# rlangefe/pygemma

Hardware: AMD Instinct MI355X
Metric: SNPs/sec (whole node) at n=10,000 c=5; K-eigendecomp wallclock (higher is better)
Workload: dtype i8x3->i32 MFMA (genotype codes exact, integer accumulation exact; U as 24-bit fixed point per eigenvector in three int8 planes) rotation + f64 Gram/sweeps (f32 rounding points of the reference)

## Files before the change

### pygemma_amd/csrc/assoc.hip

```cpp
#include "common.hpp"

#include <cmath>

namespace pg {

constexpr int NLAM = 11;
#ifndef PG_ASSOC_WPB
#define PG_ASSOC_WPB 2
#endif
constexpr int WPB = PG_ASSOC_WPB;
#define PG_MINV 1e-35f
#ifndef PG_FUSE_PQ_MAX
#define PG_FUSE_PQ_MAX 36
#endif
#ifndef PG_FUSE_PQR_MAX
#define PG_FUSE_PQR_MAX 28
#endif
#ifndef PG_PFD
#define PG_PFD 2
#endif
#ifndef PG_CHUNK_MIN_NP
#define PG_CHUNK_MIN_NP 80
#endif
#ifndef PG_SCAN_NV
#define PG_SCAN_NV 96
#endif
#ifndef PG_SWEEP_LDS_MIN_SLOTS
#define PG_SWEEP_LDS_MIN_SLOTS 3
#endif
#ifndef PG_PHENO_SPLIT_XE
#define PG_PHENO_SPLIT_XE 26
#endif
#ifndef PG_WAVES
#define PG_WAVES 2
#endif
#ifndef PG_ASSOC_FINAL_P
#define PG_ASSOC_FINAL_P 1
#endif
#ifndef PG_ASSOC_NEWTON_REUSE
#define PG_ASSOC_NEWTON_REUSE 1
#endif
#ifndef PG_REUSE_MAX_SLOTS
#define PG_REUSE_MAX_SLOTS 4
#endif
#ifndef PG_ASSOC_DECADE_HOIST
#define PG_ASSOC_DECADE_HOIST 1
#endif

__host__ __device__ constexpr size_t assoc_dtab_doubles(int c) { return (size_t)c * (c + 2) * 4 + 8; }

__host__ __device__ constexpr size_t assoc_sav_doubles(int sav_slots) { return sav_slots ? (size_t)2 * (2 * sav_slots + 1) * 64 : 0; }
__host__ __device__ constexpr size_t assoc_per_wave_bytes(int M, bool sweep_lds, int sav_slots, size_t evalout_bytes, int n_vals)
{
    return (((sweep_lds ? (size_t)3 * M * 8 : 0) + assoc_sav_doubles(sav_slots) * 8 + (size_t)NLAM * 2 * M * 8 + NLAM * evalout_bytes + 2 * NLAM * 4 +
             (size_t)n_vals * 4) + 15) & ~(size_t)15;
}

struct AssocParams {
    int n, npad, c, niter, nu, grid, rowf;
    long long p, ldx;
    const float *xr;
    const float *fixed;
    float *htab;
    double *fixg;
    double *t1tab;
    float *ldHtab;
    double *dtab;
    float lam11[NLAM];
    float logl_c;
    const int *leaf, *node, *level, *chunk;
    int n_leaf, n_level, n_chunk, n_vals;
    float *beta, *se, *tau, *lam;
    double *F;
    unsigned long long *stats;
    unsigned *trace;
    unsigned long long *passes;
    int lrt, nhalf;
    float ml_c;
    float *lalt, *lamalt;
    const double *xbuf;
    int xe, xcol;
};

struct EvalOut { float yPy, yPPy, yPPPy, trP, trPP, ld, Pxx_c, Pyx_c, sh, shh; };

__device__ __forceinline__ float hinv_f32(float lam, float d)
// ... 349 lines not shown
{
    const float4 *src = reinterpret_cast<const float4 *>(pr.fixed + (size_t)i * pr.rowf);
#pragma unroll
    for (int k = 0; k < Elem<C>::S4; k++) e.row[k] = src[k];
    const int ic = min(i, pr.n - 1);
    e.x = HASX ? xrow[ic] : 0.0f;
}
constexpr int PFD = PG_PFD;
template <class E, int PF = PFD, class LoadF, class BodyF>
__device__ __forceinline__ void pipelined(int niter, LoadF &&ld, BodyF &&body)
{
    E buf[PF];
#pragma unroll
    for (int d = 0; d < PF; d++) ld(buf[d], d < niter ? d : niter - 1);
    for (int it = 0; it < niter; it += PF) {
#pragma unroll
        for (int d = 0; d < PF; d++) {
            if (it + d < niter) body(buf[d], it + d);
            const int nx = it + d + PF;
            ld(buf[d], nx < niter ? nx : niter - 1);
        }
    }
}
template <int C>
__device__ __forceinline__ void unpack_elem(const AssocParams &pr, const Elem<C> &e, int i, float &d, float (&col)[C + 2])
{
    float buf[4 * Elem<C>::S4];
#pragma unroll
    for (int k = 0; k < Elem<C>::S4; k++) {
        buf[4 * k] = e.row[k].x; buf[4 * k + 1] = e.row[k].y; buf[4 * k + 2] = e.row[k].z; buf[4 * k + 3] = e.row[k].w;
    }
    d = buf[0];
#pragma unroll
    for (int j = 0; j < C; j++) col[j] = buf[1 + j];
    col[C] = e.x;
    col[C + 1] = buf[C + 1];
}
template <int C> struct WaldElem {
    using E = Elem<C>;
    using Row = const float *;
    template <bool HASX>
    static __device__ __forceinline__ void load(const AssocParams &pr, Row xrow, int i, E &e) { load_elem<C, HASX>(pr, xrow, i, e); }
    static __device__ __forceinline__ void unpack(const AssocParams &pr, const E &e, int i, float &d, float (&col)[C + 2]) { unpack_elem<C>(pr, e, i, d, col); }
};

template <int C, int MASK, bool HASX, class EL = WaldElem<C>>
__device__ __forceinline__ void gram_pass(const AssocParams &pr, typename EL::Row xrow, float lam, int lane, float *htab_out,
                                          double (&Po)[Shape<C>::SLOTS], double (&Qo)[Shape<C>::SLOTS], double (&Ro)[Shape<C>::SLOTS],
                                          double &t1, double &t2)
{
    constexpr int M = Shape<C>::M, NP = Shape<C>::NP;
    constexpr bool DP = (MASK & 1) != 0, DQ = (MASK & 2) != 0, DR = (MASK & 4) != 0;
    double P[DP ? NP : 1], Q[DQ ? NP : 1], R[DR ? NP : 1];
#pragma unroll
    for (int k = 0; k < NP; k++) { if constexpr (DP) P[k] = 0.0; if constexpr (DQ) Q[k] = 0.0; if constexpr (DR) R[k] = 0.0; }
    double s1 = 0.0, s2 = 0.0;
    using E = typename EL::E;
    pipelined<E>(pr.niter, [&](E &e, int it) { EL::template load<HASX>(pr, xrow, it * 64 + lane, e); },
                       [&](const E &cur, int it) {
        const int i = it * 64 + lane;
        float d, colf[M];
        EL::unpack(pr, cur, i, d, colf);
        const float h = hinv_f32(lam, d);
        if (htab_out) htab_out[i] = h;
        const double hd = (double)h;
        double col[M], a[M];
#pragma unroll
        for (int j = 0; j < M; j++) { col[j] = (double)colf[j]; a[j] = hd * col[j]; }
        if (DP || DQ) {
#pragma unroll
            for (int j = 0; j < M; j++)
#pragma unroll
                for (int k = 0; k <= j; k++) {
                    if constexpr (DP) P[tri(j, k)] = fma(a[j], col[k], P[tri(j, k)]);
                    if constexpr (DQ) Q[tri(j, k)] = fma(a[j], a[k], Q[tri(j, k)]);
                }
        }
        if (DP) s1 += hd;
        if constexpr (DR) {
            const double h2 = hd * hd;
#pragma unroll
            for (int j = 0; j < M; j++) {
                const double gj = h2 * col[j];
#pragma unroll
                for (int k = 0; k <= j; k++) R[tri(j, k)] = fma(gj, a[k], R[tri(j, k)]);
            }
            s2 = fma(hd, hd, s2);
        }
    });
    if constexpr (DP) { scatter_entries<C>(P, lane, Po); t1 = bfly(s1); }
    if constexpr (DQ) scatter_entries<C>(Q, lane, Qo);
    if constexpr (DR) { scatter_entries<C>(R, lane, Ro); t2 = bfly(s2); }
}

template <int C, int PW, int SL, bool HASX, class EL = WaldElem<C>>
__device__ __forceinline__ void gram_pass_slot(const AssocParams &pr, typename EL::Row xrow, float lam, int lane, float *htab_out, double &out, double &tsum)
{
    constexpr int M = Shape<C>::M, E0 = 64 * SL, NV = Shape<C>::slot_nv(SL), NVP = next_pow2(NV);
    double acc[NVP];
#pragma unroll
    for (int k = 0; k < NVP; k++) acc[k] = 0.0;
    double s = 0.0;
    using E = typename EL::E;
    pipelined<E, (M > 22 ? 1 : PFD)>(pr.niter, [&](E &e, int it) { EL::template load<HASX>(pr, xrow, it * 64 + lane, e); },
                       [&](const E &cur, int it) {
        const int i = it * 64 + lane;
        float d, colf[M];
        EL::unpack(pr, cur, i, d, colf);
        const float h = hinv_f32(lam, d);
        if (htab_out) htab_out[i] = h;
        const double hd = (double)h, h2 = hd * hd;
        double col[M], a[M], g[PW == 3 ? M : 1];
#pragma unroll
        for (int j = 0; j < M; j++) { col[j] = (double)colf[j]; a[j] = hd * col[j]; if constexpr (PW == 3) g[j] = h2 * col[j]; }
#pragma unroll
        for (int j = 0; j < M; j++)
#pragma unroll
            for (int k = 0; k <= j; k++) {
                const int e = tri(j, k);
                if (e >= E0 && e < E0 + NV) {
                    if constexpr (PW == 1) acc[e - E0] = fma(a[j], col[k], acc[e - E0]);
                    else if constexpr (PW == 2) acc[e - E0] = fma(a[j], a[k], acc[e - E0]);
                    else acc[e - E0] = fma(g[j], a[k], acc[e - E0]);
                }
            }
        if constexpr (SL == 0 && PW == 1) s += hd;
        if constexpr (SL == 0 && PW == 3) s = fma(hd, hd, s);
    });
    out = reduce_scatter<NVP>(acc, lane);
    if constexpr (SL == 0 && (PW == 1 || PW == 3)) tsum = bfly(s);
}
template <int C, int PW, bool HASX, int SL = 0, class EL = WaldElem<C>>
__device__ __forceinline__ void slot_passes(const AssocParams &pr, typename EL::Row xrow, float lam, int lane, float *htab_out,
                                            double (&X)[Shape<C>::SLOTS], double &tsum)
{
    gram_pass_slot<C, PW, SL, HASX, EL>(pr, xrow, lam, lane, SL == 0 ? htab_out : nullptr, X[SL], tsum);
    if constexpr (SL + 1 < Shape<C>::SLOTS) slot_passes<C, PW, HASX, SL + 1, EL>(pr, xrow, lam, lane, htab_out, X, tsum);
}

template <int C, int MASK, class EL = WaldElem<C>>
__device__ __forceinline__ void gram_powers(const AssocParams &pr, typename EL::Row xrow, float lam, int lane,
                                            double (&P)[Shape<C>::SLOTS], double (&Q)[Shape<C>::SLOTS], double (&R)[Shape<C>::SLOTS],
                                            double &t1, double &t2)
{
    constexpr bool DP = (MASK & 1) != 0, DQ = (MASK & 2) != 0, DR = (MASK & 4) != 0;
    if constexpr (Shape<C>::CHUNKED) {
        double tq = 0.0;
        if constexpr (DP) slot_passes<C, 1, true, 0, EL>(pr, xrow, lam, lane, nullptr, P, t1);
        if constexpr (DQ) slot_passes<C, 2, true, 0, EL>(pr, xrow, lam, lane, nullptr, Q, tq);
        if constexpr (DR) slot_passes<C, 3, true, 0, EL>(pr, xrow, lam, lane, nullptr, R, t2);
    } else if constexpr (MASK == PW_PQR && Shape<C>::FUSE_PQR) {
        gram_pass<C, 7, true, EL>(pr, xrow, lam, lane, nullptr, P, Q, R, t1, t2);
    } else if constexpr (DP && DQ && Shape<C>::FUSE_PQ) {
        gram_pass<C, 3, true, EL>(pr, xrow, lam, lane, nullptr, P, Q, R, t1, t2);
        if constexpr (DR) gram_pass<C, 4, true, EL>(pr, xrow, lam, lane, nullptr, P, Q, R, t1, t2);
    } else {
        if constexpr (DP) gram_pass<C, 1, true, EL>(pr, xrow, lam, lane, nullptr, P, Q, R, t1, t2);
        if constexpr (DQ) gram_pass<C, 2, true, EL>(pr, xrow, lam, lane, nullptr, P, Q, R, t1, t2);
        if constexpr (DR) gram_pass<C, 4, true, EL>(pr, xrow, lam, lane, nullptr, P, Q, R, t1, t2);
// ... 4 lines not shown
__device__ __forceinline__ void eval_specific(const AssocParams &pr, typename EL::Row xrow, float lam, int lane, const Own<C> &own, EvalOut &o,
                                              double *piv)
{
    constexpr int SLOTS = Shape<C>::SLOTS;
    double P[SLOTS], Q[SLOTS], R[SLOTS], t1 = 0.0, t2 = 0.0;
#pragma unroll
    for (int sl = 0; sl < SLOTS; sl++) { Q[sl] = 0.0; R[sl] = 0.0; }
    gram_powers<C, PW, EL>(pr, xrow, lam, lane, P, Q, R, t1, t2);
    lane_sweeps<C, PW>(P, Q, R, own, t1, t2, lane, o, piv);
}

template <int C>
__global__ __launch_bounds__(64) void setup_tabs_kernel(AssocParams pr)
{
    constexpr int NP = Shape<C>::NP, SLOTS = Shape<C>::SLOTS;
    extern __shared__ float smem_f[];
    const int t = blockIdx.x, lane = threadIdx.x;
    const float lam = pr.lam11[t];
    Own<C> own;
    own.init(lane);
    double P[SLOTS], Q[SLOTS], R[SLOTS], t1 = 0.0, t2 = 0.0;
    if constexpr (Shape<C>::CHUNKED) {
        double tq = 0.0;
        slot_passes<C, 1, false>(pr, nullptr, lam, lane, pr.htab + (size_t)t * pr.npad, P, t1);
        slot_passes<C, 2, false>(pr, nullptr, lam, lane, nullptr, Q, tq);
    } else if constexpr (Shape<C>::FUSE_PQ) {
        gram_pass<C, 3, false>(pr, nullptr, lam, lane, pr.htab + (size_t)t * pr.npad, P, Q, R, t1, t2);
    } else {
        gram_pass<C, 1, false>(pr, nullptr, lam, lane, pr.htab + (size_t)t * pr.npad, P, Q, R, t1, t2);
        gram_pass<C, 2, false>(pr, nullptr, lam, lane, nullptr, P, Q, R, t1, t2);
    }
#pragma unroll
    for (int sl = 0; sl < SLOTS; sl++)
        if (own.valid[sl]) {
            pr.fixg[((size_t)t * 2 + 0) * NP + own.e[sl]] = P[sl];
            pr.fixg[((size_t)t * 2 + 1) * NP + own.e[sl]] = Q[sl];
        }
    float ldH = device_logdet_H(pr, lam, lane, smem_f);
    if (lane == 0) { pr.t1tab[t] = t1; pr.ldHtab[t] = ldH; }
    if constexpr (PG_ASSOC_DECADE_HOIST && C >= 1) {
        __shared__ double piv_s[Shape<C>::SWEEP_LDS ? 3 * Shape<C>::M : 1];
        if (pr.dtab) {
            double *rec = pr.dtab + (size_t)t * assoc_dtab_doubles(C);
            EvalOut e;
            lane_sweeps<C, PW_PQ, true>(P, Q, R, own, t1, 0.0, lane, e, piv_s, rec);
            double *tail = rec + (size_t)C * Shape<C>::M * 4;
            if (lane == 0) { tail[4] = t1; tail[5] = (double)ldH; tail[6] = (double)lam; tail[7] = 0.0; }
        }
    }
}

template <int C, int GG>
__device__ __forceinline__ void scan_accumulate(const AssocParams &pr, const float *xrow, int t0, int lane, double *xent)
{
    constexpr int M = Shape<C>::M, NV = GG * 2 * M;
    constexpr int NV0 = NV < 64 ? NV : 64, NV1 = NV > 64 ? NV - 64 : 0;
    constexpr int NVP0 = next_pow2(NV0), NVP1 = next_pow2(NV1 > 0 ? NV1 : 1);
    static_assert(NV <= 128, "scan group too large");
    double acc[NV0 == 64 ? 64 + NVP1 : NVP0];
#pragma unroll
    for (int k = 0; k < (NV0 == 64 ? 64 + NVP1 : NVP0); k++) acc[k] = 0.0;
    struct SE { Elem<C> e; float h[GG]; };
    pipelined<SE>(pr.niter, [&](SE &q, int it) {
        const int i = it * 64 + lane;
        load_elem<C>(pr, xrow, i, q.e);
#pragma unroll
        for (int g = 0; g < GG; g++) q.h[g] = pr.htab[(size_t)(t0 + g) * pr.npad + i];
    }, [&](const SE &q, int it) {
        const int i = it * 64 + lane;
        float d, colf[M];
        unpack_elem<C>(pr, q.e, i, d, colf);
        const double xd = (double)colf[C];
        double z[M];
#pragma unroll
        for (int k = 0; k <= C; k++) z[k] = xd * (double)colf[k];
        z[C + 1] = (double)colf[C + 1] * xd;
#pragma unroll
        for (int g = 0; g < GG; g++) {
            const double hd = (double)q.h[g];
            const double h2 = hd * hd;
#pragma unroll
            for (int k = 0; k <= C + 1; k++) {
                acc[g * 2 * M + k] = fma(hd, z[k], acc[g * 2 * M + k]);
                acc[g * 2 * M + M + k] = fma(h2, z[k], acc[g * 2 * M + M + k]);
            }
        }
    });
    {
        double t[NVP0];
#pragma unroll
        for (int k = 0; k < NVP0; k++) t[k] = acc[k];
        const double tot = reduce_scatter<NVP0>(t, lane);
        const int idx = lane % NVP0;
        if (idx < NV0 && lane < NVP0) xent[t0 * 2 * M + idx] = tot;
    }
    if constexpr (NV1 > 0) {
        double t[NVP1];
#pragma unroll
        for (int k = 0; k < NVP1; k++) t[k] = acc[64 + k];
        const double tot = reduce_scatter<NVP1>(t, lane);
        const int idx = lane % NVP1;
        if (idx < NV1 && lane < NVP1) xent[t0 * 2 * M + 64 + idx] = tot;
    }
}
template <int C, int T0>
__device__ __forceinline__ void scan_all(const AssocParams &pr, const float *xrow, int lane, double *xent)
{
    constexpr int G = Shape<C>::G;
    if constexpr (T0 < NLAM) {
        constexpr int GG = (NLAM - T0) < G ? (NLAM - T0) : G;
        scan_accumulate<C, GG>(pr, xrow, T0, lane, xent);
        scan_all<C, T0 + GG>(pr, xrow, lane, xent);
    }
}

template <int C, int TC, int GG, int PWS, int PW0>
__device__ __forceinline__ void scan_pheno_accumulate(const AssocParams &pr, const float *xrow, const float *Y, long long ldy, int tcn,
                                                      int t0, int lane, double *out)
{
    constexpr int M = Shape<C>::M, XE = C + 1 + TC, NV = GG * PWS * XE;
    auto dest = [&](int v) { const int gg = v / (PWS * XE), r = v - gg * PWS * XE; return (t0 + gg) * 2 * XE + PW0 * XE + r; };
    constexpr int NV0 = NV < 64 ? NV : 64, NV1 = NV > 64 ? NV - 64 : 0;
    constexpr int NVP0 = next_pow2(NV0), NVP1 = next_pow2(NV1 > 0 ? NV1 : 1);
    static_assert(NV <= 128, "scan group too large");
    double acc[NV0 == 64 ? 64 + NVP1 : NVP0];
#pragma unroll
    for (int k = 0; k < (NV0 == 64 ? 64 + NVP1 : NVP0); k++) acc[k] = 0.0;
    struct SE { Elem<C> e; float y[TC]; float h[GG]; };
    pipelined<SE>(pr.niter, [&](SE &q, int it) {
        const int i = it * 64 + lane;
        load_elem<C>(pr, xrow, i, q.e);
#pragma unroll
        for (int j = 0; j < TC; j++) q.y[j] = (i < pr.n && j < tcn) ? Y[(size_t)j * ldy + i] : 0.0f;
#pragma unroll
        for (int g = 0; g < GG; g++) q.h[g] = pr.htab[(size_t)(t0 + g) * pr.npad + i];
    }, [&](const SE &q, int it) {
        const int i = it * 64 + lane;
        float d, colf[M];
        unpack_elem<C>(pr, q.e, i, d, colf);
        const double xd = (double)colf[C];
        double z[XE];
#pragma unroll
        for (int k = 0; k <= C; k++) z[k] = xd * (double)colf[k];
#pragma unroll
        for (int j = 0; j < TC; j++) z[C + 1 + j] = (double)q.y[j] * xd;
#pragma unroll
        for (int g = 0; g < GG; g++) {
            const double hd = (double)q.h[g];
            const double h2 = hd * hd;
#pragma unroll
            for (int k = 0; k < XE; k++) {
                if constexpr (PWS == 2) {
                    acc[g * 2 * XE + k] = fma(hd, z[k], acc[g * 2 * XE + k]);
                    acc[g * 2 * XE + XE + k] = fma(h2, z[k], acc[g * 2 * XE + XE + k]);
                } else {
                    acc[g * XE + k] = fma(PW0 == 0 ? hd : h2, z[k], acc[g * XE + k]);
                }
            }
// ... 5 lines not shown
        for (int k = 0; k < NVP0; k++) t[k] = acc[k];
        const double tot = reduce_scatter<NVP0>(t, lane);
        const int idx = lane % NVP0;
        if (idx < NV0 && lane < NVP0) out[dest(idx)] = tot;
    }
    if constexpr (NV1 > 0) {
        double t[NVP1];
#pragma unroll
        for (int k = 0; k < NVP1; k++) t[k] = acc[64 + k];
        const double tot = reduce_scatter<NVP1>(t, lane);
        const int idx = lane % NVP1;
        if (idx < NV1 && lane < NVP1) out[dest(64 + idx)] = tot;
    }
}
template <int C, int TC, int T0>
__device__ __forceinline__ void scan_pheno_all(const AssocParams &pr, const float *xrow, const float *Y, long long ldy, int tcn, int lane,
                                               double *out)
{
    constexpr int XE = C + 1 + TC, PWS = XE > PG_PHENO_SPLIT_XE ? 1 : 2;
    constexpr int G0 = PWS == 1 ? 1 : (Shape<C>::SCAN_NV - XE) / (PWS * XE), G = G0 < 1 ? 1 : (G0 > NLAM ? NLAM : G0);
    if constexpr (T0 < NLAM) {
        constexpr int GG = (NLAM - T0) < G ? (NLAM - T0) : G;
        if constexpr (PWS == 2) {
            scan_pheno_accumulate<C, TC, GG, 2, 0>(pr, xrow, Y, ldy, tcn, T0, lane, out);
        } else {
            scan_pheno_accumulate<C, TC, GG, 1, 0>(pr, xrow, Y, ldy, tcn, T0, lane, out);
            scan_pheno_accumulate<C, TC, GG, 1, 1>(pr, xrow, Y, ldy, tcn, T0, lane, out);
        }
        scan_pheno_all<C, TC, T0 + GG>(pr, xrow, Y, ldy, tcn, lane, out);
    }
}
constexpr int SCAN_WPB = 4;
template <int C, int TC>
__global__ __launch_bounds__(64 * SCAN_WPB, PG_WAVES) void scan_pheno_kernel(AssocParams pr, const float *Y, long long ldy, int tcn, double *xbuf)
{
    const int wave = threadIdx.x >> 6, lane = threadIdx.x & 63;
    const long long g = (long long)blockIdx.x * SCAN_WPB + wave;
    if (g >= pr.p) return;
    scan_pheno_all<C, TC, 0>(pr, pr.xr + (size_t)g * pr.ldx, Y, ldy, tcn, lane, xbuf + (size_t)g * NLAM * 2 * (C + 1 + TC));
}

__device__ __forceinline__ void wave_lds_sync()
{
    __builtin_amdgcn_fence(__ATOMIC_RELEASE, "wavefront");
    __builtin_amdgcn_wave_barrier();
    __builtin_amdgcn_fence(__ATOMIC_ACQUIRE, "wavefront");
}

template <class Fn>
__device__ __forceinline__ double brentq_dev(Fn &&f, double xa, double xb, double fa, double fb, int maxiter = 100)
// ... 316 lines not shown
            atomicAdd(&pr.passes[2], (unsigned long long)n_full); atomicAdd(&pr.passes[3], (unsigned long long)n_reuse);
        }
    }
    ASSOC_STAMP(3);
}

#if defined(PG_ASSOC_PART) && (PG_ASSOC_PART == 6 || PG_ASSOC_PART == 7)
struct GxeRows { const float *x, *xe; };
template <int CS> struct GxeVals {
    static constexpr int S4 = (CS + 2 + 3) / 4;
    float4 row[S4];
    float x, xe;
};
template <int C> struct GxeElem {
    static constexpr int CS = C - 1;
    using E = GxeVals<CS>;
    using Row = GxeRows;
    template <bool HASX>
    static __device__ __forceinline__ void load(const AssocParams &pr, Row r, int i, E &e)
    {
        const float4 *src = reinterpret_cast<const float4 *>(pr.fixed + (size_t)i * pr.rowf);
#pragma unroll
        for (int k = 0; k < E::S4; k++) e.row[k] = src[k];
        const int ic = min(i, pr.n - 1);
        e.x = r.x[ic];
        e.xe = r.xe[ic];
    }
    static __device__ __forceinline__ void unpack(const AssocParams &pr, const E &e, int i, float &d, float (&col)[C + 2])
    {
        float buf[4 * E::S4];
#pragma unroll
        for (int k = 0; k < E::S4; k++) {
            buf[4 * k] = e.row[k].x; buf[4 * k + 1] = e.row[k].y; buf[4 * k + 2] = e.row[k].z; buf[4 * k + 3] = e.row[k].w;
        }
        d = buf[0];
#pragma unroll
        for (int j = 0; j < CS; j++) col[j] = buf[1 + j];
        col[CS] = e.x;
        col[CS + 1] = e.xe;
        col[CS + 2] = buf[CS + 1];
    }
};
template <int CS> struct GxeShape {
    static constexpr int C = CS + 1, NE = 2 * CS + 5;
    static constexpr int PWS = NE > PG_PHENO_SPLIT_XE ? 1 : 2;
    static constexpr int G0 = (Shape<C>::SCAN_NV - NE) / (PWS * NE), G = G0 < 1 ? 1 : (G0 > NLAM ? NLAM : G0);
};
__host__ __device__ constexpr size_t gxe_per_wave_bytes(int M, bool sweep_lds, int NE, size_t evalout_bytes, int n_vals)
{
    return (((sweep_lds ? (size_t)3 * M * 8 : 0) + (size_t)NLAM * 2 * NE * 8 + NLAM * evalout_bytes + 2 * NLAM * 4 + (size_t)n_vals * 4) + 15) & ~(size_t)15;
}

template <int CS, int GG, int PWS, int PW0>
__device__ __forceinline__ void gxe_scan_accumulate(const AssocParams &pr, GxeRows xr, int t0, int lane, double *out)
{
    using EL = GxeElem<CS + 1>;
    constexpr int M = CS + 3, NE = GxeShape<CS>::NE, NV = GG * PWS * NE;
    auto dest = [&](int v) { const int gg = v / (PWS * NE), r = v - gg * PWS * NE; return (t0 + gg) * 2 * NE + PW0 * NE + r; };
    constexpr int NV0 = NV < 64 ? NV : 64, NV1 = NV > 64 ? NV - 64 : 0;
    constexpr int NVP0 = next_pow2(NV0), NVP1 = next_pow2(NV1 > 0 ? NV1 : 1);
    static_assert(NV <= 128, "scan group too large");
    double acc[NV0 == 64 ? 64 + NVP1 : NVP0];
#pragma unroll
    for (int k = 0; k < (NV0 == 64 ? 64 + NVP1 : NVP0); k++) acc[k] = 0.0;
    struct SE { typename EL::E e; float h[GG]; };
    pipelined<SE>(pr.niter, [&](SE &q, int it) {
        const int i = it * 64 + lane;
        EL::template load<true>(pr, xr, i, q.e);
#pragma unroll
        for (int g = 0; g < GG; g++) q.h[g] = pr.htab[(size_t)(t0 + g) * pr.npad + i];
    }, [&](const SE &q, int it) {
        const int i = it * 64 + lane;
        float d, colf[M];
        EL::unpack(pr, q.e, i, d, colf);
        const double xd = (double)colf[CS], ed = (double)colf[CS + 1], yd = (double)colf[CS + 2];
        double z[NE];
#pragma unroll
        for (int k = 0; k < CS; k++) { z[k] = xd * (double)colf[k]; z[CS + 1 + k] = ed * (double)colf[k]; }
        z[CS] = xd * xd;
        z[2 * CS + 1] = ed * xd;
        z[2 * CS + 2] = ed * ed;
        z[2 * CS + 3] = yd * xd;
        z[2 * CS + 4] = yd * ed;
#pragma unroll
        for (int g = 0; g < GG; g++) {
            const double hd = (double)q.h[g];
            const double h2 = hd * hd;
#pragma unroll
            for (int k = 0; k < NE; k++) {
                if constexpr (PWS == 2) {
                    acc[g * 2 * NE + k] = fma(hd, z[k], acc[g * 2 * NE + k]);
                    acc[g * 2 * NE + NE + k] = fma(h2, z[k], acc[g * 2 * NE + NE + k]);
                } else {
                    acc[g * NE + k] = fma(PW0 == 0 ? hd : h2, z[k], acc[g * NE + k]);
                }
            }
        }
// ... 2 lines not shown
        double t[NVP0];
#pragma unroll
        for (int k = 0; k < NVP0; k++) t[k] = acc[k];
        const double tot = reduce_scatter<NVP0>(t, lane);
        const int idx = lane % NVP0;
        if (idx < NV0 && lane < NVP0) out[dest(idx)] = tot;
    }
    if constexpr (NV1 > 0) {
        double t[NVP1];
#pragma unroll
        for (int k = 0; k < NVP1; k++) t[k] = acc[64 + k];
        const double tot = reduce_scatter<NVP1>(t, lane);
        const int idx = lane % NVP1;
        if (idx < NV1 && lane < NVP1) out[dest(64 + idx)] = tot;
    }
}
template <int CS, int T0>
__device__ __forceinline__ void gxe_scan_all(const AssocParams &pr, GxeRows xr, int lane, double *xent)
{
    constexpr int G = GxeShape<CS>::G;
    if constexpr (T0 < NLAM) {
        constexpr int GG = (NLAM - T0) < G ? (NLAM - T0) : G;
        if constexpr (GxeShape<CS>::PWS == 2) {
            gxe_scan_accumulate<CS, GG, 2, 0>(pr, xr, T0, lane, xent);
        } else {
            gxe_scan_accumulate<CS, GG, 1, 0>(pr, xr, T0, lane, xent);
            gxe_scan_accumulate<CS, GG, 1, 1>(pr, xr, T0, lane, xent);
        }
        gxe_scan_all<CS, T0 + GG>(pr, xr, lane, xent);
    }
}

template <int CS>
__global__ __launch_bounds__(64 * WPB, PG_WAVES) void assoc_gxe_kernel(AssocParams pr, const float *xer, long long ldxe)
{
    constexpr int C = CS + 1, M = Shape<C>::M, SLOTS = Shape<C>::SLOTS, NE = GxeShape<CS>::NE, NPS = Shape<CS>::NP;
    using EL = GxeElem<C>;
    extern __shared__ unsigned char smem[];
    const int wave = threadIdx.x >> 6, lane = threadIdx.x & 63;
    const long long g = (long long)blockIdx.x * WPB + wave;
    if (g >= pr.p) return;
    constexpr size_t piv_bytes = Shape<C>::SWEEP_LDS ? (size_t)3 * M * 8 : 0;
    unsigned char *base = smem + (size_t)wave * gxe_per_wave_bytes(M, Shape<C>::SWEEP_LDS, NE, sizeof(EvalOut), pr.n_vals);
    double *piv = reinterpret_cast<double *>(base);
    base += piv_bytes;
    double *xent = reinterpret_cast<double *>(base);
    EvalOut *evs = reinterpret_cast<EvalOut *>(base + (size_t)NLAM * 2 * NE * 8);
    float *d1s = reinterpret_cast<float *>(evs + NLAM);
    float *lls = d1s + NLAM;
    float *vals = lls + NLAM;
// ... 529 lines not shown
    {
        float r = (float)((double)(n / 2) * std::log((double)n / (2.0 * M_PI)));
        pr.ml_c = r - (float)(n / 2);
    }
    pr.leaf = ctx->plan.d_leaf; pr.node = ctx->plan.d_node; pr.level = ctx->plan.d_level; pr.chunk = ctx->plan.d_chunk;
    pr.n_leaf = ctx->plan.n_leaf; pr.n_level = ctx->plan.n_level; pr.n_chunk = ctx->plan.n_chunk;
    pr.n_vals = ctx->plan.n_leaf + ctx->plan.n_node;
}

static int assoc_run(pg_ctx *ctx, int64_t n, int c, int64_t p, const float *d, const float *Wr, int64_t ldw, const float *yr,
                     const float *Xr, int64_t ldx, int grid, float *beta, float *se, float *tau, float *lambda, double *F,
                     unsigned long long *stats_dev, bool lrt, float *lalt, float *lamalt)
{
    PG_HIP(hipSetDevice(ctx->device));
    int rc = build_npsum_plan(ctx, n);
    if (rc) return rc;

    AssocParams pr{};
    fill_params(ctx, n, c, grid, pr);
    pr.p = p; pr.ldx = ldx; pr.xr = Xr;
    const int M = c + 2, NP = M * (M + 1) / 2;
    rc = ensure(ctx, &ctx->fixed, &ctx->fixed_bytes, (size_t)pr.npad * pr.rowf * 4);
    if (rc) return rc;
    const size_t off_fixg = ((size_t)NLAM * pr.npad * 4 + 255) & ~(size_t)255;
    const size_t off_t1 = off_fixg + (size_t)NLAM * 2 * NP * 8;
    const size_t off_ldh = off_t1 + NLAM * 8;
    const size_t off_dtab = (off_ldh + NLAM * 4 + 255) & ~(size_t)255;
    rc = ensure(ctx, &ctx->tabs, &ctx->tabs_bytes, off_dtab + NLAM * assoc_dtab_doubles(c) * 8 + 256);
    if (rc) return rc;
    if (!ctx->stats) PG_HIP(hipMalloc(&ctx->stats, 16));
    pr.fixed = (const float *)ctx->fixed;
    pr.htab = (float *)ctx->tabs;
    pr.fixg = (double *)((char *)ctx->tabs + off_fixg);
    pr.t1tab = (double *)((char *)ctx->tabs + off_t1);
    pr.ldHtab = (float *)((char *)ctx->tabs + off_ldh);
    pr.dtab = (double *)((char *)ctx->tabs + off_dtab);
    pr.lrt = lrt ? 1 : 0;
    pr.lalt = lalt; pr.lamalt = lamalt;
    pr.beta = beta; pr.se = se; pr.tau = tau; pr.lam = lambda; pr.F = F;
    pr.stats = stats_dev;
    pr.trace = lrt ? nullptr : ctx->eval_trace;
    pr.passes = lrt ? nullptr : ctx->pass_stats;

    build_fixed_kernel<<<(pr.npad + 255) / 256, 256, 0, ctx->stream>>>(pr.n, pr.npad, c, (int)ldw, pr.rowf, d, Wr, yr, (float *)ctx->fixed);
    PG_HIP(hipGetLastError());
    return launch_assoc_any(ctx, pr);
}

extern "C" int pg_assoc_dev(pg_ctx *ctx, int64_t n, int c, int64_t p, const float *d, const float *Wr, const float *yr,
                            const float *Xr, int64_t ldx, int grid, float *beta, float *se, float *tau, float *lambda,
                            double *F, double *pval, unsigned long long *stats_dev)
{
    PG_REQUIRE(ctx && d && Wr && yr && Xr && beta && se && tau && lambda && F, "pg_assoc_dev: NULL argument");
    PG_REQUIRE(n >= 2 && n < (1LL << 30) && p >= 0 && ldx >= n, "pg_assoc_dev: bad shape n=%lld p=%lld ldx=%lld", (long long)n, (long long)p, (long long)ldx);
    if (c < 1 || c > PG_MAX_COVARIATES) {
// ... 1 lines not shown
        return PG_ENOTSUP;
    }
    PG_REQUIRE(n - c - 1 > 0, "pg_assoc_dev: n - c - 1 must be positive");
    if (p == 0) return PG_OK;
    int rc = assoc_run(ctx, n, c, p, d, Wr, c, yr, Xr, ldx, grid, beta, se, tau, lambda, F, stats_dev, false, nullptr, nullptr);
    if (rc) return rc;
    if (pval) return pg_fdist_sf_dev(ctx, p, F, (double)(n - c - 1), pval);
    return PG_OK;
}

extern "C" int pg_assoc_warm(pg_ctx *ctx, int64_t n, int c)
{
    PG_REQUIRE(ctx && n >= 2 && n < (1LL << 30), "pg_assoc_warm: bad arguments");
    if (c < 1 || c > PG_MAX_COVARIATES) {
        set_error("pg_assoc_warm: c=%d covariates not supported by this build (1..%d)", c, PG_MAX_COVARIATES);
        return PG_ENOTSUP;
    }
    PG_HIP(hipSetDevice(ctx->device));
    int rc = build_npsum_plan(ctx, n);
    if (rc) return rc;
    const int npad = (int)((n + 63) / 64 * 64), rowf = ((c + 2 + 3) / 4) * 4, M = c + 2, NP = M * (M + 1) / 2;
    rc = ensure(ctx, &ctx->fixed, &ctx->fixed_bytes, (size_t)npad * rowf * 4);
    if (rc) return rc;
    const size_t off_fixg = ((size_t)NLAM * npad * 4 + 255) & ~(size_t)255;
    rc = ensure(ctx, &ctx->tabs, &ctx->tabs_bytes,
                ((off_fixg + (size_t)NLAM * 2 * NP * 8 + NLAM * 8 + NLAM * 4 + 255) & ~(size_t)255) + NLAM * assoc_dtab_doubles(c) * 8 + 256);
    if (rc) return rc;
    if (!ctx->stats) PG_HIP(hipMalloc(&ctx->stats, 16));
    return PG_OK;
}

extern "C" int pg_assoc_set_eval_trace(pg_ctx *ctx, unsigned *trace_dev)
{
    PG_REQUIRE(ctx, "pg_assoc_set_eval_trace: NULL ctx");
    ctx->eval_trace = trace_dev;
    return PG_OK;
}

extern "C" int pg_assoc_set_pass_stats(pg_ctx *ctx, unsigned long long *dev4)
{
    PG_REQUIRE(ctx, "pg_assoc_set_pass_stats: NULL ctx");
    ctx->pass_stats = dev4;
    return PG_OK;
}

#ifdef PG_ASSOC_STAMPS
extern "C" int pgx_assoc_stamps(long long *out4096)
{
    return hipMemcpyFromSymbol(out4096, HIP_SYMBOL(pg::g_assoc_stamps), sizeof(long long) * 4096) == hipSuccess ? 0 : -1;
}
#endif

struct PhenoLayout {
    int npad, rowf, NP, tpad_max;
    long long ptile;
    size_t off_htab, off_fixg, off_t1, off_ldh, off_xbuf, bytes;
};
static PhenoLayout pheno_layout(int64_t n, int c, int t, int64_t p)
{
    PhenoLayout L{};
    auto up = [](size_t v) { return (v + 255) & ~(size_t)255; };
    L.npad = (int)((n + 63) / 64 * 64); L.rowf = ((c + 2 + 3) / 4) * 4; L.NP = (c + 2) * (c + 3) / 2;
    const int tc = t < PHENO_CHUNK ? t : PHENO_CHUNK;
    L.tpad_max = 1;
    while (L.tpad_max < tc) L.tpad_max <<= 1;
    const size_t per_snp = (size_t)NLAM * 2 * (c + 1 + L.tpad_max) * 8;
    const long long cap = (long long)((256u << 20) / per_snp);
    L.ptile = p < cap ? p : (cap < 1024 ? 1024 : cap);
    if (L.ptile > p) L.ptile = p;
    L.off_htab = up((size_t)PHENO_CHUNK * L.npad * L.rowf * 4);
    L.off_fixg = L.off_htab + up((size_t)NLAM * L.npad * 4);
    L.off_t1 = L.off_fixg + up((size_t)PHENO_CHUNK * NLAM * 2 * L.NP * 8);
    L.off_ldh = L.off_t1 + up(NLAM * 8);
    L.off_xbuf = L.off_ldh + up(NLAM * 4);
    L.bytes = L.off_xbuf + up((size_t)L.ptile * per_snp);
    return L;
}

extern "C" int pg_assoc_pheno_dev(pg_ctx *ctx, int64_t n, int c, int64_t p, int t, const float *d, const float *Wr,
                                  const float *Yr, int64_t ldy, const float *Xr, int64_t ldx, int grid,
                                  float *beta, float *se, float *tau, float *lambda, double *F, double *pval,
                                  unsigned long long *stats_dev)
{
    PG_REQUIRE(ctx && d && Wr && Yr && Xr && beta && se && tau && lambda && F, "pg_assoc_pheno_dev: NULL argument");
    PG_REQUIRE(n >= 2 && n < (1LL << 30) && p >= 0 && ldx >= n, "pg_assoc_pheno_dev: bad shape n=%lld p=%lld ldx=%lld",
               (long long)n, (long long)p, (long long)ldx);
    if (c < 1 || c > PG_MAX_COVARIATES) {
        set_error("pg_assoc_pheno_dev: c=%d covariates not supported by this build (1..%d)", c, PG_MAX_COVARIATES);
        return PG_ENOTSUP;
    }
    PG_REQUIRE(n - c - 1 > 0, "pg_assoc_pheno_dev: n - c - 1 must be positive");
    PG_REQUIRE(t >= 1 && ldy >= n, "pg_assoc_pheno_dev: bad phenotypes t=%d ldy=%lld (n=%lld)", t, (long long)ldy, (long long)n);
    if (p == 0) return PG_OK;
    PG_HIP(hipSetDevice(ctx->device));
    int rc = build_npsum_plan(ctx, n);
    if (rc) return rc;
    const PhenoLayout L = pheno_layout(n, c, t, p);
    rc = ensure(ctx, &ctx->pheno, &ctx->pheno_bytes, L.bytes);
    if (rc) return rc;
    char *base = (char *)ctx->pheno;
    float *fixed = (float *)base;
    double *fixg = (double *)(base + L.off_fixg), *xbuf = (double *)(base + L.off_xbuf);

    AssocParams pr{};
    fill_params(ctx, n, c, grid, pr);
    pr.ldx = ldx;
    pr.htab = (float *)(base + L.off_htab);
    pr.t1tab = (double *)(base + L.off_t1);
    pr.ldHtab = (float *)(base + L.off_ldh);
    pr.stats = stats_dev;
    const size_t fixed_stride = (size_t)L.npad * L.rowf, fixg_stride = (size_t)NLAM * 2 * L.NP;
    for (int k0 = 0; k0 < t; k0 += PHENO_CHUNK) {
        const int tcn = (t - k0) < PHENO_CHUNK ? (t - k0) : PHENO_CHUNK;
        int tpad = 1;
        while (tpad < tcn) tpad <<= 1;
        for (int j = 0; j < tcn; j++) {
            pr.fixed = fixed + j * fixed_stride;
            pr.fixg = fixg + j * fixg_stride;
            build_fixed_kernel<<<(L.npad + 255) / 256, 256, 0, ctx->stream>>>(pr.n, L.npad, c, c, L.rowf, d, Wr, Yr + (size_t)(k0 + j) * ldy,
                                                                             (float *)pr.fixed);
            PG_HIP(hipGetLastError());
            rc = launch_assoc_pheno(ctx, pr, PhenoLaunch{PhenoLaunch::SETUP, nullptr, 0, 0, 0, nullptr});
            if (rc) return rc;
        }
        pr.xe = c + 1 + tpad; pr.xbuf = xbuf;
        for (int64_t s0 = 0; s0 < p; s0 += L.ptile) {
            pr.p = (p - s0) < L.ptile ? (p - s0) : L.ptile;
            pr.xr = Xr + (size_t)s0 * ldx;
            rc = launch_assoc_pheno(ctx, pr, PhenoLaunch{PhenoLaunch::SCAN, Yr + (size_t)k0 * ldy, ldy, tcn, tpad, xbuf});
            if (rc) return rc;
// ... 26 lines not shown
extern "C" int pg_assoc_gxe_dev(pg_ctx *ctx, int64_t n, int c, int64_t p, const float *d, const float *Wr, const float *yr,
                                const float *xr, int64_t ldx, const float *xer, int64_t ldxe, float *beta, float *se, float *tau,
                                float *lambda, double *F, double *pval, unsigned long long *stats_dev)
{
    PG_REQUIRE(ctx && d && Wr && yr && xr && xer && beta && se && tau && lambda && F, "pg_assoc_gxe_dev: NULL argument");
    PG_REQUIRE(n >= 2 && n < (1LL << 30) && p >= 0 && ldx >= n && ldxe >= n, "pg_assoc_gxe_dev: bad shape n=%lld p=%lld ldx=%lld ldxe=%lld",
               (long long)n, (long long)p, (long long)ldx, (long long)ldxe);
    if (c < 1 || c + 1 > PG_MAX_COVARIATES) {
        set_error("pg_assoc_gxe_dev: c=%d shared covariates not supported by this build (1..%d)", c, PG_MAX_COVARIATES - 1);
        return PG_ENOTSUP;
    }
    PG_REQUIRE(n - c - 2 > 0, "pg_assoc_gxe_dev: n - c - 2 must be positive");
    if (p == 0) return PG_OK;
    PG_HIP(hipSetDevice(ctx->device));
    int rc = build_npsum_plan(ctx, n);
    if (rc) return rc;
    AssocParams pr{};
    fill_params(ctx, n, c + 1, 0, pr);
    pr.c = c; pr.rowf = ((c + 2 + 3) / 4) * 4;
    pr.p = p; pr.ldx = ldx; pr.xr = xr;
    const int NP = (c + 2) * (c + 3) / 2;
    rc = ensure(ctx, &ctx->fixed, &ctx->fixed_bytes, (size_t)pr.npad * pr.rowf * 4);
    if (rc) return rc;
    const size_t off_fixg = ((size_t)NLAM * pr.npad * 4 + 255) & ~(size_t)255;
    const size_t off_t1 = off_fixg + (size_t)NLAM * 2 * NP * 8;
    const size_t off_ldh = off_t1 + NLAM * 8;
    rc = ensure(ctx, &ctx->tabs, &ctx->tabs_bytes, off_ldh + NLAM * 4 + 256);
    if (rc) return rc;
    pr.fixed = (const float *)ctx->fixed;
    pr.htab = (float *)ctx->tabs;
    pr.fixg = (double *)((char *)ctx->tabs + off_fixg);
    pr.t1tab = (double *)((char *)ctx->tabs + off_t1);
    pr.ldHtab = (float *)((char *)ctx->tabs + off_ldh);
    pr.beta = beta; pr.se = se; pr.tau = tau; pr.lam = lambda; pr.F = F;
    pr.stats = stats_dev;
    build_fixed_kernel<<<(pr.npad + 255) / 256, 256, 0, ctx->stream>>>(pr.n, pr.npad, c, c, pr.rowf, d, Wr, yr, (float *)ctx->fixed);
    PG_HIP(hipGetLastError());
    rc = launch_assoc_gxe(ctx, pr, xer, ldxe);
    if (rc) return rc;
    if (pval) return pg_fdist_sf_dev(ctx, p, F, (double)(n - c - 2), pval);
    return PG_OK;
}

extern "C" int pg_assoc_gxe_warm(pg_ctx *ctx, int64_t n, int c)
{
    PG_REQUIRE(ctx && n >= 2 && n < (1LL << 30), "pg_assoc_gxe_warm: bad arguments");
    if (c < 1 || c + 1 > PG_MAX_COVARIATES) {
        set_error("pg_assoc_gxe_warm: c=%d shared covariates not supported by this build (1..%d)", c, PG_MAX_COVARIATES - 1);
        return PG_ENOTSUP;
    }
    return pg_assoc_warm(ctx, n, c);
}

// ... 168 lines not shown
```

Baseline: 1.945 million.

## Interleave lambda weight table per element and deepen genotype prefetch ring in scans

Stores the per-lambda h table element-major (12 floats per sample) for small covariate counts, so a scan group reads its lambdas with float4/float2 vector loads instead of strided scalar loads. The genotype x values are also prefetched through a separate, deeper ring (4 iterations) than the fixed-row/h-table loads, which aims to hide global latency on the genotype stream. The cost is a larger table allocation, more live registers for the ring, and a layout flag that every writer and reader has to respect.

```diff
diff --git a/pygemma_amd/csrc/assoc.hip b/pygemma_amd/csrc/assoc.hip
--- a/pygemma_amd/csrc/assoc.hip
+++ b/pygemma_amd/csrc/assoc.hip
@@ -18,6 +18,9 @@
 #endif
 #ifndef PG_PFD
 #define PG_PFD 2
+#endif
+#ifndef PG_SCAN_XPF
+#define PG_SCAN_XPF 4
 #endif
 #ifndef PG_CHUNK_MIN_NP
 #define PG_CHUNK_MIN_NP 80
@@ -56,12 +59,59 @@
              (size_t)n_vals * 4) + 15) & ~(size_t)15;
 }
 
+constexpr int HROW = 12;
+__host__ __device__ constexpr size_t htab_bytes(int npad) { return (size_t)npad * HROW * 4; }
+__device__ __forceinline__ float *htab_entry(float *htab, int npad, bool elem, int t, int i)
+{
+    return elem ? htab + (size_t)i * HROW + t : htab + (size_t)t * npad + i;
+}
+struct HtabCol {
+    float *p = nullptr;
+    int step = 0;
+    HtabCol() = default;
+    __host__ __device__ HtabCol(decltype(nullptr)) {}
+    __device__ HtabCol(float *htab, int npad, bool elem, int t) : p(htab_entry(htab, npad, elem, t, 0)), step(elem ? HROW : 1) {}
+    __device__ __forceinline__ void put(int i, float h) const { if (p) p[(size_t)i * step] = h; }
+};
+template <int T0, int GG, int G = 0>
+__device__ __forceinline__ void htab_load_row(const float *hrow, float (&h)[GG])
+{
+    static_assert(T0 >= 0 && T0 + GG <= NLAM && NLAM < HROW && HROW % 4 == 0, "a group of decade lambdas");
+    if constexpr (G < GG) {
+        constexpr int off = T0 + G, rem = GG - G;
+        if constexpr (off % 4 == 0 && (rem >= 4 || (rem == 3 && off + 4 == HROW))) {
+            const float4 v = *reinterpret_cast<const float4 *>(hrow + off);
+            h[G] = v.x; h[G + 1] = v.y; h[G + 2] = v.z;
+            if constexpr (rem >= 4) h[G + 3] = v.w;
+            htab_load_row<T0, GG, G + 4>(hrow, h);
+        } else if constexpr (off % 2 == 0 && rem >= 2) {
+            const float2 v = *reinterpret_cast<const float2 *>(hrow + off);
+            h[G] = v.x; h[G + 1] = v.y;
+            htab_load_row<T0, GG, G + 2>(hrow, h);
+        } else {
+            h[G] = hrow[off];
+            htab_load_row<T0, GG, G + 1>(hrow, h);
+        }
+    }
+}
+template <bool ELEM, int T0, int GG>
+__device__ __forceinline__ void htab_load(float *htab, int npad, int i, float (&h)[GG])
+{
+    if constexpr (ELEM) {
+        htab_load_row<T0, GG>(htab_entry(htab, npad, true, 0, i), h);
+    } else {
+#pragma unroll
+        for (int g = 0; g < GG; g++) h[g] = *htab_entry(htab, npad, false, T0 + g, i);
+    }
+}
+
 struct AssocParams {
     int n, npad, c, niter, nu, grid, rowf;
     long long p, ldx;
     const float *xr;
     const float *fixed;
     float *htab;
+    int helem;
     double *fixg;
     double *t1tab;
     float *ldHtab;
@@ -457,6 +507,49 @@
         }
     }
 }
+constexpr int SCAN_XPF = PG_SCAN_XPF;
+template <class E, class X, int XPF = SCAN_XPF, int PF = PFD, class LoadF, class LoadXF, class BodyF>
+__device__ __forceinline__ void pipelined_x(int niter, LoadF &&ld, LoadXF &&ldx, BodyF &&body)
+{
+    static_assert(XPF >= PF && XPF % PF == 0, "the x ring is a whole number of table rings deep");
+    E buf[PF];
+    X xq[XPF];
+#pragma unroll
+    for (int d = 0; d < XPF; d++) ldx(xq[d], d < niter ? d : niter - 1);
+#pragma unroll
+    for (int d = 0; d < PF; d++) ld(buf[d], d < niter ? d : niter - 1);
+    int it = 0;
+    for (; it + XPF <= niter; it += XPF) {
+#pragma unroll
+        for (int d = 0; d < XPF; d++) {
+            body(buf[d % PF], xq[d], it + d);
+            const int nt = it + d + PF, nx = it + d + XPF;
+            ld(buf[d % PF], nt < niter ? nt : niter - 1);
+            ldx(xq[d], nx < niter ? nx : niter - 1);
+        }
+    }
+#pragma unroll
+    for (int d = 0; d + 1 < XPF; d++)
+        if (it + d < niter) {
+            body(buf[d % PF], xq[d], it + d);
+            const int nt = it + d + PF;
+            if (d + PF + 1 < XPF) ld(buf[d % PF], nt < niter ? nt : niter - 1);
+        }
+}
+#ifndef PG_SCAN_RING_MAX_M
+#define PG_SCAN_RING_MAX_M 8
+#endif
+__host__ __device__ constexpr bool scan_ring(int M) { return M <= PG_SCAN_RING_MAX_M; }
+template <bool RING, class E, class X, class LoadF, class LoadXF, class BodyF>
+__device__ __forceinline__ void scan_pipelined(int niter, LoadF &&ld, LoadXF &&ldx, BodyF &&body)
+{
+    if constexpr (RING) {
+        pipelined_x<E, X>(niter, ld, ldx, body);
+    } else {
+        struct EX { E e; X x; };
+        pipelined<EX>(niter, [&](EX &q, int it) { ld(q.e, it); ldx(q.x, it); }, [&](const EX &q, int it) { body(q.e, q.x, it); });
+    }
+}
 template <int C>
 __device__ __forceinline__ void unpack_elem(const AssocParams &pr, const Elem<C> &e, int i, float &d, float (&col)[C + 2])
 {
@@ -480,7 +573,7 @@
 };
 
 template <int C, int MASK, bool HASX, class EL = WaldElem<C>>
-__device__ __forceinline__ void gram_pass(const AssocParams &pr, typename EL::Row xrow, float lam, int lane, float *htab_out,
+__device__ __forceinline__ void gram_pass(const AssocParams &pr, typename EL::Row xrow, float lam, int lane, HtabCol htab_out,
                                           double (&Po)[Shape<C>::SLOTS], double (&Qo)[Shape<C>::SLOTS], double (&Ro)[Shape<C>::SLOTS],
                                           double &t1, double &t2)
 {
@@ -497,7 +590,7 @@
         float d, colf[M];
         EL::unpack(pr, cur, i, d, colf);
         const float h = hinv_f32(lam, d);
-        if (htab_out) htab_out[i] = h;
+        htab_out.put(i, h);
         const double hd = (double)h;
         double col[M], a[M];
 #pragma unroll
@@ -529,7 +622,7 @@
 }
 
 template <int C, int PW, int SL, bool HASX, class EL = WaldElem<C>>
-__device__ __forceinline__ void gram_pass_slot(const AssocParams &pr, typename EL::Row xrow, float lam, int lane, float *htab_out, double &out, double &tsum)
+__device__ __forceinline__ void gram_pass_slot(const AssocParams &pr, typename EL::Row xrow, float lam, int lane, HtabCol htab_out, double &out, double &tsum)
 {
     constexpr int M = Shape<C>::M, E0 = 64 * SL, NV = Shape<C>::slot_nv(SL), NVP = next_pow2(NV);
     double acc[NVP];
@@ -543,7 +636,7 @@
         float d, colf[M];
         EL::unpack(pr, cur, i, d, colf);
         const float h = hinv_f32(lam, d);
-        if (htab_out) htab_out[i] = h;
+        htab_out.put(i, h);
         const double hd = (double)h, h2 = hd * hd;
         double col[M], a[M], g[PW == 3 ? M : 1];
 #pragma unroll
@@ -566,10 +659,10 @@
     if constexpr (SL == 0 && (PW == 1 || PW == 3)) tsum = bfly(s);
 }
 template <int C, int PW, bool HASX, int SL = 0, class EL = WaldElem<C>>
-__device__ __forceinline__ void slot_passes(const AssocParams &pr, typename EL::Row xrow, float lam, int lane, float *htab_out,
+__device__ __forceinline__ void slot_passes(const AssocParams &pr, typename EL::Row xrow, float lam, int lane, HtabCol htab_out,
                                             double (&X)[Shape<C>::SLOTS], double &tsum)
 {
-    gram_pass_slot<C, PW, SL, HASX, EL>(pr, xrow, lam, lane, SL == 0 ? htab_out : nullptr, X[SL], tsum);
+    gram_pass_slot<C, PW, SL, HASX, EL>(pr, xrow, lam, lane, SL == 0 ? htab_out : HtabCol(), X[SL], tsum);
     if constexpr (SL + 1 < Shape<C>::SLOTS) slot_passes<C, PW, HASX, SL + 1, EL>(pr, xrow, lam, lane, htab_out, X, tsum);
 }
 
@@ -620,12 +713,12 @@
     double P[SLOTS], Q[SLOTS], R[SLOTS], t1 = 0.0, t2 = 0.0;
     if constexpr (Shape<C>::CHUNKED) {
         double tq = 0.0;
-        slot_passes<C, 1, false>(pr, nullptr, lam, lane, pr.htab + (size_t)t * pr.npad, P, t1);
+        slot_passes<C, 1, false>(pr, nullptr, lam, lane, HtabCol(pr.htab, pr.npad, pr.helem != 0, t), P, t1);
         slot_passes<C, 2, false>(pr, nullptr, lam, lane, nullptr, Q, tq);
     } else if constexpr (Shape<C>::FUSE_PQ) {
-        gram_pass<C, 3, false>(pr, nullptr, lam, lane, pr.htab + (size_t)t * pr.npad, P, Q, R, t1, t2);
+        gram_pass<C, 3, false>(pr, nullptr, lam, lane, HtabCol(pr.htab, pr.npad, pr.helem != 0, t), P, Q, R, t1, t2);
     } else {
-        gram_pass<C, 1, false>(pr, nullptr, lam, lane, pr.htab + (size_t)t * pr.npad, P, Q, R, t1, t2);
+        gram_pass<C, 1, false>(pr, nullptr, lam, lane, HtabCol(pr.htab, pr.npad, pr.helem != 0, t), P, Q, R, t1, t2);
         gram_pass<C, 2, false>(pr, nullptr, lam, lane, nullptr, P, Q, R, t1, t2);
     }
 #pragma unroll
@@ -634,6 +727,8 @@
             pr.fixg[((size_t)t * 2 + 0) * NP + own.e[sl]] = P[sl];
             pr.fixg[((size_t)t * 2 + 1) * NP + own.e[sl]] = Q[sl];
         }
+    if (pr.helem && t == NLAM - 1)
+        for (int i = lane; i < pr.npad; i += 64) *htab_entry(pr.htab, pr.npad, true, NLAM, i) = 0.0f;
     float ldH = device_logdet_H(pr, lam, lane, smem_f);
     if (lane == 0) { pr.t1tab[t] = t1; pr.ldHtab[t] = ldH; }
     if constexpr (PG_ASSOC_DECADE_HOIST && C >= 1) {
@@ -648,8 +743,8 @@
     }
 }
 
-template <int C, int GG>
-__device__ __forceinline__ void scan_accumulate(const AssocParams &pr, const float *xrow, int t0, int lane, double *xent)
+template <int C, int T0, int GG>
+__device__ __forceinline__ void scan_accumulate(const AssocParams &pr, const float *xrow, int lane, double *xent)
 {
     constexpr int M = Shape<C>::M, NV = GG * 2 * M;
     constexpr int NV0 = NV < 64 ? NV : 64, NV1 = NV > 64 ? NV - 64 : 0;
@@ -659,15 +754,16 @@
 #pragma unroll
     for (int k = 0; k < (NV0 == 64 ? 64 + NVP1 : NVP0); k++) acc[k] = 0.0;
     struct SE { Elem<C> e; float h[GG]; };
-    pipelined<SE>(pr.niter, [&](SE &q, int it) {
+    scan_pipelined<scan_ring(M), SE, float>(pr.niter, [&](SE &q, int it) {
         const int i = it * 64 + lane;
-        load_elem<C>(pr, xrow, i, q.e);
-#pragma unroll
-        for (int g = 0; g < GG; g++) q.h[g] = pr.htab[(size_t)(t0 + g) * pr.npad + i];
-    }, [&](const SE &q, int it) {
+        load_elem<C, false>(pr, nullptr, i, q.e);
+        htab_load<scan_ring(M), T0, GG>(pr.htab, pr.npad, i, q.h);
+    }, [&](float &x, int it) { x = xrow[min(it * 64 + lane, pr.n - 1)]; },
+    [&](const SE &q, float x, int it) {
         const int i = it * 64 + lane;
         float d, colf[M];
         unpack_elem<C>(pr, q.e, i, d, colf);
+        colf[C] = x;
         const double xd = (double)colf[C];
         double z[M];
 #pragma unroll
@@ -690,7 +786,7 @@
         for (int k = 0; k < NVP0; k++) t[k] = acc[k];
         const double tot = reduce_scatter<NVP0>(t, lane);
         const int idx = lane % NVP0;
-        if (idx < NV0 && lane < NVP0) xent[t0 * 2 * M + idx] = tot;
+        if (idx < NV0 && lane < NVP0) xent[T0 * 2 * M + idx] = tot;
     }
     if constexpr (NV1 > 0) {
         double t[NVP1];
@@ -698,7 +794,7 @@
         for (int k = 0; k < NVP1; k++) t[k] = acc[64 + k];
         const double tot = reduce_scatter<NVP1>(t, lane);
         const int idx = lane % NVP1;
-        if (idx < NV1 && lane < NVP1) xent[t0 * 2 * M + 64 + idx] = tot;
+        if (idx < NV1 && lane < NVP1) xent[T0 * 2 * M + 64 + idx] = tot;
     }
 }
 template <int C, int T0>
@@ -707,17 +803,17 @@
     constexpr int G = Shape<C>::G;
     if constexpr (T0 < NLAM) {
         constexpr int GG = (NLAM - T0) < G ? (NLAM - T0) : G;
-        scan_accumulate<C, GG>(pr, xrow, T0, lane, xent);
+        scan_accumulate<C, T0, GG>(pr, xrow, lane, xent);
         scan_all<C, T0 + GG>(pr, xrow, lane, xent);
     }
 }
 
-template <int C, int TC, int GG, int PWS, int PW0>
+template <int C, int TC, int T0, int GG, int PWS, int PW0>
 __device__ __forceinline__ void scan_pheno_accumulate(const AssocParams &pr, const float *xrow, const float *Y, long long ldy, int tcn,
-                                                      int t0, int lane, double *out)
+                                                      int lane, double *out)
 {
     constexpr int M = Shape<C>::M, XE = C + 1 + TC, NV = GG * PWS * XE;
-    auto dest = [&](int v) { const int gg = v / (PWS * XE), r = v - gg * PWS * XE; return (t0 + gg) * 2 * XE + PW0 * XE + r; };
+    auto dest = [&](int v) { const int gg = v / (PWS * XE), r = v - gg * PWS * XE; return (T0 + gg) * 2 * XE + PW0 * XE + r; };
     constexpr int NV0 = NV < 64 ? NV : 64, NV1 = NV > 64 ? NV - 64 : 0;
     constexpr int NVP0 = next_pow2(NV0), NVP1 = next_pow2(NV1 > 0 ? NV1 : 1);
     static_assert(NV <= 128, "scan group too large");
@@ -730,8 +826,7 @@
         load_elem<C>(pr, xrow, i, q.e);
 #pragma unroll
         for (int j = 0; j < TC; j++) q.y[j] = (i < pr.n && j < tcn) ? Y[(size_t)j * ldy + i] : 0.0f;
-#pragma unroll
-        for (int g = 0; g < GG; g++) q.h[g] = pr.htab[(size_t)(t0 + g) * pr.npad + i];
+        htab_load<false, T0, GG>(pr.htab, pr.npad, i, q.h);
     }, [&](const SE &q, int it) {
         const int i = it * 64 + lane;
         float d, colf[M];
@@ -783,10 +878,10 @@
     if constexpr (T0 < NLAM) {
         constexpr int GG = (NLAM - T0) < G ? (NLAM - T0) : G;
         if constexpr (PWS == 2) {
-            scan_pheno_accumulate<C, TC, GG, 2, 0>(pr, xrow, Y, ldy, tcn, T0, lane, out);
+            scan_pheno_accumulate<C, TC, T0, GG, 2, 0>(pr, xrow, Y, ldy, tcn, lane, out);
         } else {
-            scan_pheno_accumulate<C, TC, GG, 1, 0>(pr, xrow, Y, ldy, tcn, T0, lane, out);
-            scan_pheno_accumulate<C, TC, GG, 1, 1>(pr, xrow, Y, ldy, tcn, T0, lane, out);
+            scan_pheno_accumulate<C, TC, T0, GG, 1, 0>(pr, xrow, Y, ldy, tcn, lane, out);
+            scan_pheno_accumulate<C, TC, T0, GG, 1, 1>(pr, xrow, Y, ldy, tcn, lane, out);
         }
         scan_pheno_all<C, TC, T0 + GG>(pr, xrow, Y, ldy, tcn, lane, out);
     }
@@ -1149,9 +1244,14 @@
         const float4 *src = reinterpret_cast<const float4 *>(pr.fixed + (size_t)i * pr.rowf);
 #pragma unroll
         for (int k = 0; k < E::S4; k++) e.row[k] = src[k];
+        if constexpr (HASX) load_x(pr, r, i, e.x, e.xe);
+        else { e.x = 0.0f; e.xe = 0.0f; }
+    }
+    static __device__ __forceinline__ void load_x(const AssocParams &pr, Row r, int i, float &x, float &xe)
+    {
         const int ic = min(i, pr.n - 1);
-        e.x = r.x[ic];
-        e.xe = r.xe[ic];
+        x = r.x[ic];
+        xe = r.xe[ic];
     }
     static __device__ __forceinline__ void unpack(const AssocParams &pr, const E &e, int i, float &d, float (&col)[C + 2])
     {
@@ -1178,12 +1278,12 @@
     return (((sweep_lds ? (size_t)3 * M * 8 : 0) + (size_t)NLAM * 2 * NE * 8 + NLAM * evalout_bytes + 2 * NLAM * 4 + (size_t)n_vals * 4) + 15) & ~(size_t)15;
 }
 
-template <int CS, int GG, int PWS, int PW0>
-__device__ __forceinline__ void gxe_scan_accumulate(const AssocParams &pr, GxeRows xr, int t0, int lane, double *out)
+template <int CS, int T0, int GG, int PWS, int PW0>
+__device__ __forceinline__ void gxe_scan_accumulate(const AssocParams &pr, GxeRows xr, int lane, double *out)
 {
     using EL = GxeElem<CS + 1>;
     constexpr int M = CS + 3, NE = GxeShape<CS>::NE, NV = GG * PWS * NE;
-    auto dest = [&](int v) { const int gg = v / (PWS * NE), r = v - gg * PWS * NE; return (t0 + gg) * 2 * NE + PW0 * NE + r; };
+    auto dest = [&](int v) { const int gg = v / (PWS * NE), r = v - gg * PWS * NE; return (T0 + gg) * 2 * NE + PW0 * NE + r; };
     constexpr int NV0 = NV < 64 ? NV : 64, NV1 = NV > 64 ? NV - 64 : 0;
     constexpr int NVP0 = next_pow2(NV0), NVP1 = next_pow2(NV1 > 0 ? NV1 : 1);
     static_assert(NV <= 128, "scan group too large");
@@ -1191,15 +1291,17 @@
 #pragma unroll
     for (int k = 0; k < (NV0 == 64 ? 64 + NVP1 : NVP0); k++) acc[k] = 0.0;
     struct SE { typename EL::E e; float h[GG]; };
-    pipelined<SE>(pr.niter, [&](SE &q, int it) {
+    struct XS { float x, xe; };
+    scan_pipelined<scan_ring(M), SE, XS>(pr.niter, [&](SE &q, int it) {
         const int i = it * 64 + lane;
-        EL::template load<true>(pr, xr, i, q.e);
-#pragma unroll
-        for (int g = 0; g < GG; g++) q.h[g] = pr.htab[(size_t)(t0 + g) * pr.npad + i];
-    }, [&](const SE &q, int it) {
+        EL::template load<false>(pr, xr, i, q.e);
+        htab_load<scan_ring(M), T0, GG>(pr.htab, pr.npad, i, q.h);
+    }, [&](XS &s, int it) { EL::load_x(pr, xr, it * 64 + lane, s.x, s.xe); },
+    [&](const SE &q, const XS &s, int it) {
         const int i = it * 64 + lane;
         float d, colf[M];
         EL::unpack(pr, q.e, i, d, colf);
+        colf[CS] = s.x; colf[CS + 1] = s.xe;
         const double xd = (double)colf[CS], ed = (double)colf[CS + 1], yd = (double)colf[CS + 2];
         double z[NE];
 #pragma unroll
@@ -1248,10 +1350,10 @@
     if constexpr (T0 < NLAM) {
         constexpr int GG = (NLAM - T0) < G ? (NLAM - T0) : G;
         if constexpr (GxeShape<CS>::PWS == 2) {
-            gxe_scan_accumulate<CS, GG, 2, 0>(pr, xr, T0, lane, xent);
+            gxe_scan_accumulate<CS, T0, GG, 2, 0>(pr, xr, lane, xent);
         } else {
-            gxe_scan_accumulate<CS, GG, 1, 0>(pr, xr, T0, lane, xent);
-            gxe_scan_accumulate<CS, GG, 1, 1>(pr, xr, T0, lane, xent);
+            gxe_scan_accumulate<CS, T0, GG, 1, 0>(pr, xr, lane, xent);
+            gxe_scan_accumulate<CS, T0, GG, 1, 1>(pr, xr, lane, xent);
         }
         gxe_scan_all<CS, T0 + GG>(pr, xr, lane, xent);
     }
@@ -1827,7 +1929,7 @@
     const int M = c + 2, NP = M * (M + 1) / 2;
     rc = ensure(ctx, &ctx->fixed, &ctx->fixed_bytes, (size_t)pr.npad * pr.rowf * 4);
     if (rc) return rc;
-    const size_t off_fixg = ((size_t)NLAM * pr.npad * 4 + 255) & ~(size_t)255;
+    const size_t off_fixg = (htab_bytes(pr.npad) + 255) & ~(size_t)255;
     const size_t off_t1 = off_fixg + (size_t)NLAM * 2 * NP * 8;
     const size_t off_ldh = off_t1 + NLAM * 8;
     const size_t off_dtab = (off_ldh + NLAM * 4 + 255) & ~(size_t)255;
@@ -1835,7 +1937,7 @@
     if (rc) return rc;
     if (!ctx->stats) PG_HIP(hipMalloc(&ctx->stats, 16));
     pr.fixed = (const float *)ctx->fixed;
-    pr.htab = (float *)ctx->tabs;
+    pr.htab = (float *)ctx->tabs;  pr.helem = scan_ring(c + 2);
     pr.fixg = (double *)((char *)ctx->tabs + off_fixg);
     pr.t1tab = (double *)((char *)ctx->tabs + off_t1);
     pr.ldHtab = (float *)((char *)ctx->tabs + off_ldh);
@@ -1883,7 +1985,7 @@
     const int npad = (int)((n + 63) / 64 * 64), rowf = ((c + 2 + 3) / 4) * 4, M = c + 2, NP = M * (M + 1) / 2;
     rc = ensure(ctx, &ctx->fixed, &ctx->fixed_bytes, (size_t)npad * rowf * 4);
     if (rc) return rc;
-    const size_t off_fixg = ((size_t)NLAM * npad * 4 + 255) & ~(size_t)255;
+    const size_t off_fixg = (htab_bytes(npad) + 255) & ~(size_t)255;
     rc = ensure(ctx, &ctx->tabs, &ctx->tabs_bytes,
                 ((off_fixg + (size_t)NLAM * 2 * NP * 8 + NLAM * 8 + NLAM * 4 + 255) & ~(size_t)255) + NLAM * assoc_dtab_doubles(c) * 8 + 256);
     if (rc) return rc;
@@ -1930,7 +2032,7 @@
     L.ptile = p < cap ? p : (cap < 1024 ? 1024 : cap);
     if (L.ptile > p) L.ptile = p;
     L.off_htab = up((size_t)PHENO_CHUNK * L.npad * L.rowf * 4);
-    L.off_fixg = L.off_htab + up((size_t)NLAM * L.npad * 4);
+    L.off_fixg = L.off_htab + up(htab_bytes(L.npad));
     L.off_t1 = L.off_fixg + up((size_t)PHENO_CHUNK * NLAM * 2 * L.NP * 8);
     L.off_ldh = L.off_t1 + up(NLAM * 8);
     L.off_xbuf = L.off_ldh + up(NLAM * 4);
@@ -1966,7 +2068,7 @@
     AssocParams pr{};
     fill_params(ctx, n, c, grid, pr);
     pr.ldx = ldx;
-    pr.htab = (float *)(base + L.off_htab);
+    pr.htab = (float *)(base + L.off_htab);  pr.helem = 0;
     pr.t1tab = (double *)(base + L.off_t1);
     pr.ldHtab = (float *)(base + L.off_ldh);
     pr.stats = stats_dev;
@@ -2039,13 +2141,13 @@
     const int NP = (c + 2) * (c + 3) / 2;
     rc = ensure(ctx, &ctx->fixed, &ctx->fixed_bytes, (size_t)pr.npad * pr.rowf * 4);
     if (rc) return rc;
-    const size_t off_fixg = ((size_t)NLAM * pr.npad * 4 + 255) & ~(size_t)255;
+    const size_t off_fixg = (htab_bytes(pr.npad) + 255) & ~(size_t)255;
     const size_t off_t1 = off_fixg + (size_t)NLAM * 2 * NP * 8;
     const size_t off_ldh = off_t1 + NLAM * 8;
     rc = ensure(ctx, &ctx->tabs, &ctx->tabs_bytes, off_ldh + NLAM * 4 + 256);
     if (rc) return rc;
     pr.fixed = (const float *)ctx->fixed;
-    pr.htab = (float *)ctx->tabs;
+    pr.htab = (float *)ctx->tabs;  pr.helem = scan_ring(c + 3);
     pr.fixg = (double *)((char *)ctx->tabs + off_fixg);
     pr.t1tab = (double *)((char *)ctx->tabs + off_t1);
     pr.ldHtab = (float *)((char *)ctx->tabs + off_ldh);
```

After: 1.985 million (median of 6 runs). +2.0%, better.
